# liuQuan98/EYOC

Measured on AMD Instinct MI355X. Metric: registered pairs/sec (30k-voxel KITTI pairs), higher is better.
Workload: dtype f32 (split16 products: fp32 storage/accumulation, 3 fp16 MFMAs on hi/lo-split operands per product); 1 GPU; 64 synthetic 30 cm KITTI-shaped pairs per step per GPU (mean 29894 voxels/cloud, ResUNetBN2C random-init, 5000-point NN, RANSAC 4000000 hypotheses/pair, planted inlier ratio 0.3, spconv math split16); parallelism=pairs sharded over 1 GPU(s), steps_in_flight=2

## Files before the change

### eyoc_amd/_lib.py

```python
from __future__ import annotations

import ctypes as C
import os
import threading

_HERE = os.path.dirname(os.path.abspath(__file__))
LIB_PATH = os.environ.get("EYOC_HIP_LIB") or os.path.join(_HERE, "lib", "libeyoc_hip.so")

MAX_LEVELS = 4
MAP_S1, MAP_DOWN, MAP_UP = 0, 1, 2


class MapsInfo(C.Structure):
    _fields_ = [("n_levels", C.c_int32), ("rows", C.c_int32 * MAX_LEVELS),
                ("pairs_s1", C.c_int64 * MAX_LEVELS), ("pairs_down", C.c_int64 * MAX_LEVELS),
                ("pairs_up", C.c_int64 * MAX_LEVELS), ("pairs_conv1", C.c_int64)]


class ModelDesc(C.Structure):
    _fields_ = [("in_channels", C.c_int32), ("out_channels", C.c_int32), ("conv1_kernel_size", C.c_int32),
                ("normalize_feature", C.c_int32), ("channels", C.c_int32 * 5), ("tr_channels", C.c_int32 * 5),
                ("bn_eps", C.c_float), ("expanded", C.c_int32)]


# ... 147 lines not shown
    "eyoc_split16_decode": (_i, [_vp, _vp, _i, _i, _i, _vp, _i, _vp]),
    "eyoc_model_set_math": (_i, [_vp, _i]),
    "eyoc_model_last_math": (_i, [_vp]),
    "eyoc_model_range_check": (_i, [_vp, _vp, C.POINTER(C.c_float)]),
    "eyoc_model_range_snapshot": (_i, [_vp, _vp, _vp]),
    "eyoc_model_set_progress_event": (_i, [_vp, _i, _vp]),
    "eyoc_model_set_probe": (_i, [_vp, _i]),
    "eyoc_spconv": (_i, [_vp, _vp, _i, _i, _vp, _i, _i, _vp, _i, _vp, _vp, _i, _i, _vp, _i, _vp]),
    "eyoc_spconv_sum": (_i, [_vp, _vp, _i, _i, _vp, _i, _i, _vp, _i, _vp, _i, _vp]),
    "eyoc_model_blob_floats": (_sz, [C.POINTER(ModelDesc)]),
    "eyoc_model_pack_host": (_i, [C.POINTER(ModelDesc), C.POINTER(LayerParams), _i, _vp, _sz]),
    "eyoc_model_create": (_i, [_vp, C.POINTER(ModelDesc), C.POINTER(LayerParams), _i, _vp, _sz, C.POINTER(_vp)]),
    "eyoc_model_blob_floats_in": (_sz, [C.POINTER(ModelDesc), _i]),
    "eyoc_model_pack_host_in": (_i, [C.POINTER(ModelDesc), C.POINTER(LayerParams), _i, _vp, _sz, _i]),
    "eyoc_model_create_in": (_i, [_vp, C.POINTER(ModelDesc), C.POINTER(LayerParams), _i, _vp, _sz, _i, C.POINTER(_vp)]),
    "eyoc_model_destroy": (_i, [_vp]),
    "eyoc_model_repack_workspace_bytes": (_sz, [_vp]),
    "eyoc_model_repack_device": (_i, [_vp, _vp, C.POINTER(LayerParams), _i, _vp, _sz, _vp]),
    "eyoc_model_fuse_tail": (_i, [_vp, _i]),
    "eyoc_model_workspace_bytes": (_sz, [_vp, _vp]),
    "eyoc_model_forward": (_i, [_vp, _vp, _vp, _vp, _vp, _vp, _sz, _vp]),
    "eyoc_model_workspace_bytes_rows": (_sz, [_vp, _vp, _i]),
    "eyoc_model_forward_rows": (_i, [_vp, _vp, _vp, _vp, _vp, _i, _vp, _vp, _sz, _vp]),
    "eyoc_model_sampled_tail": (_i, [_vp, _i]),
    "eyoc_model_num_layers": (_i, [_vp]),
    "eyoc_model_layer_work": (_i, [_vp, _vp, _vp, _vp, C.POINTER(C.c_char_p), C.POINTER(C.c_int64),
                                   C.POINTER(C.c_double), C.POINTER(C.c_double), C.POINTER(C.c_double)]),
    "eyoc_model_set_timing": (_i, [_vp, _i]),
    "eyoc_model_layer_ms": (_i, [_vp, C.POINTER(C.c_float)]),
    "eyoc_model_timing_slot": (_i, [_vp, _i]),
    "eyoc_bn_workspace_bytes": (_sz, [_i, _i]),
    "eyoc_bn_train_forward": (_i, [_vp, _vp, _i, _i, _i, _vp, _vp, C.c_float, _i, _vp, _i, _vp, _vp, _sz, _vp]),
    "eyoc_bn_train_forward_running": (_i, [_vp, _vp, _i, _i, _i, _vp, _vp, C.c_float, _i, _vp, _i, _vp, _vp, _vp, C.c_float, _vp, _sz, _vp]),
    "eyoc_bn_train_backward": (_i, [_vp, _vp, _i, _vp, _i, _vp, _i, _i, _i, _vp, _vp, C.c_float, _vp, _i, _vp, _vp, _vp, _sz, _vp]),
    "eyoc_in_chunk_rows": (_i, []),
    "eyoc_in_plan_bytes": (_sz, [_i, _i]),
    "eyoc_in_plan_layout": (_i, [_i, _i, C.POINTER(C.c_int64)]),
    "eyoc_in_plan_build": (_i, [_vp, _vp, _i, _i, _vp, _sz, _vp]),
    "eyoc_in_workspace_bytes": (_sz, [_i, _i, _i]),
    "eyoc_in_forward": (_i, [_vp, _vp, _i, _i, _i, _vp, _i, _vp, _vp, C.c_float, _i, _vp, _i, _vp, _i, _vp, _vp, _sz, _vp]),
    "eyoc_in_forward_split16": (_i, [_vp, _vp, _i, _i, _i, _vp, _i, _vp, _vp, C.c_float, _i, _vp, _i, _vp, _i, _vp, _vp, _vp, _sz, _vp]),
    "eyoc_in_backward": (_i, [_vp, _vp, _i, _vp, _i, _vp, _i, _i, _i, _vp, _i, _vp, _vp, C.c_float, _vp, _i, _vp, _i, _vp, _vp, _vp, _sz,
                              _vp]),
    "eyoc_maps_gather_window": (_i, [_vp, _vp, _i, _vp, _i, _vp, _vp]),
    "eyoc_maps_gather_window_internal": (_i, [_vp, _vp, _i, _vp, _i, _vp, _vp]),
    "eyoc_knn_prefilter": (_i, [_vp, _i]),
    "eyoc_spconv_select_up_kernel": (_i, [_vp, _i]),
    "eyoc_spconv_upc_min_rows": (_i, [_vp, _i]),
    "eyoc_spconv_upc_tile_rows": (_i, [_i, _i]),
    "eyoc_spconv_upc_bytes": (_sz, [_i]),
    "eyoc_spconv_upc_build": (_i, [_vp, _vp, _i, _vp, _vp, _vp]),
    "eyoc_spconv_upc": (_i, [_vp, _vp, _vp, _i, _i, _vp, _i, _i, _vp, _i, _vp, _i, _vp, _i, _i, _vp, _vp]),
    "eyoc_spconv_select_conv1_kernel": (_i, [_vp, _i]),
    "eyoc_knn1": (_i, [_vp, _vp, _vp, _i, C.POINTER(C.c_int32), C.POINTER(C.c_int32), _i, _i, _vp, _vp, _vp]),
    "eyoc_pdist": (_i, [_vp, _vp, _i, _vp, _i, _i, _i, _vp, _vp]),
    "eyoc_kabsch_batched": (_i, [_vp, _vp, _vp, _vp, _i, _i, _vp, _vp]),
    "eyoc_irls_quad": (_i, [_vp, _vp, _vp, _vp, _i, _i, _vp, _vp]),
    "eyoc_irls_quad_batched": (_i, [_vp, _vp, _vp, _vp, _vp, C.POINTER(C.c_int32), C.POINTER(C.c_int32), _i, _i, _vp, _vp]),
    "eyoc_valid_metrics_batched": (_i, [_vp, _vp, _vp, _vp, C.POINTER(C.c_int32), C.POINTER(C.c_int32), _vp, C.POINTER(C.c_int32), _i, _vp, _vp,
                                        C.c_double, C.c_double, _vp, _vp]),
    "eyoc_ransac": (_i, [_vp, _vp, _vp, _vp, _i, C.POINTER(RansacParams), _vp, _vp]),
    "eyoc_maps_select_orders": (_i, [_vp, _i, _i]),
    "eyoc_ransac_select_pruning": (_i, [_vp, _i]),
    "eyoc_ransac_select_generate": (_i, [_vp, _i]),
    "eyoc_knn_pack_targets": (_i, [_vp, _vp, C.POINTER(C.c_int32), _i, _i, _vp, _sz, _vp, _vp]),
    "eyoc_registration_accept_degenerate": (_i, [_vp, _i]),
    "eyoc_ransac_transform_store": (_i, [_vp, _i]),
    "eyoc_ransac_workspace_bytes": (_sz, [_vp, _i, _i, _i, _sz]),
    "eyoc_ransac_batched_ws": (_i, [_vp, _vp, _vp, _vp, C.POINTER(C.c_int32), C.POINTER(C.c_int32), _i,
                                    C.POINTER(RansacParams), _vp, _vp, _sz, _vp]),
    "eyoc_ransac_batched": (_i, [_vp, _vp, _vp, _vp, C.POINTER(C.c_int32), C.POINTER(C.c_int32), _i,
                                 C.POINTER(RansacParams), _vp, _vp]),
    "eyoc_sc2pcr_workspace_bytes": (_sz, [_i, C.POINTER(Sc2pcrParams)]),
    "eyoc_sc2pcr": (_i, [_vp, _vp, _vp, _i, C.POINTER(Sc2pcrParams), _vp, _vp, _vp, _sz, _vp]),
    "eyoc_sc2pcr_batched_workspace_bytes": (_sz, [_i, C.POINTER(Sc2pcrParams)]),
    "eyoc_sc2pcr_batched_workspace_bytes_n": (_sz, [_i, _i, C.POINTER(Sc2pcrParams)]),
    "eyoc_sc2pcr_set_shortlist_cap": (_i, [_vp, _i]),
    "eyoc_sc2pcr_set_dense_threshold": (_i, [_vp, _i]),
    "eyoc_sc2pcr_select_kernels": (_i, [_vp, _i]),
    "eyoc_sc2pcr_workspace_layout": (_i, [_i, C.POINTER(Sc2pcrParams), C.POINTER(Sc2pcrLayout)]),
    "eyoc_sc2pcr_batched": (_i, [_vp, _vp, _vp, C.POINTER(C.c_int32), _i, C.POINTER(Sc2pcrParams), _vp, _vp, _i, _vp, _sz,
                                 _vp]),
    "eyoc_icp_workspace_bytes": (_sz, [_i, _i, _i]),
    "eyoc_icp_batched": (_i, [_vp, _vp, _vp, C.POINTER(C.c_int32), C.POINTER(C.c_int32), _i, _vp, C.POINTER(IcpParams), _vp, _vp,
                              _vp, _sz, _vp]),
    "eyoc_icp_correspondences": (_i, [_vp, _vp, _vp, C.POINTER(C.c_int32), C.POINTER(C.c_int32), _i, _vp, C.c_double, _vp, _vp,
                                      _vp, _vp, _sz, _vp]),
    "eyoc_posed_nn_grid_workspace_bytes": (_sz, [_i, _i, _i]),
    "eyoc_posed_nn_grid": (_i, [_vp, _vp, _vp, C.POINTER(C.c_int32), C.POINTER(C.c_int32), _i, _vp, C.c_float, _vp, C.POINTER(C.c_int32), _vp,
                                _vp, _vp, _vp, _sz, _vp]),
    "eyoc_radius_matches_workspace_bytes": (_sz, [_i, _i, _i]),
    "eyoc_radius_matches_count": (_i, [_vp, _vp, _vp, C.POINTER(C.c_int32), C.POINTER(C.c_int32), _i, _vp, C.c_double, _i, _vp, _vp,
                                       _vp, _sz, _vp]),
    "eyoc_radius_matches_fill": (_i, [_vp, _vp, _vp, C.POINTER(C.c_int32), C.POINTER(C.c_int32), _i, _vp, C.c_double, _i, _vp, _vp,
                                      C.c_int64, _vp, _vp, _vp, _sz, _vp]),
    "eyoc_cloud_centroids_workspace_bytes": (_sz, [_i, _i]),
    "eyoc_cloud_centroids": (_i, [_vp, _vp, _i, C.POINTER(C.c_int64), _i, _i, _vp, _vp, _sz, _vp]),
    "eyoc_augment_poses": (_i, [_vp, _vp, _vp, _vp, _vp, _i, _vp, _vp, _vp]),
    "eyoc_voxelize_batched_posed_workspace_bytes": (_sz, [_i, _i]),
    "eyoc_voxelize_batched_posed": (_i, [_vp, _vp, _i, C.POINTER(C.c_int64), _i, _i, _vp, _vp, C.c_double, _i, _vp, _vp, _vp,
                                         C.POINTER(C.c_int64), _vp, _sz, _vp, _vp]),
    "eyoc_hcloss_workspace_bytes": (_sz, [_i, _i, _i, _i, _i]),
    "eyoc_hcloss_workspace_layout": (_i, [_i, _i, _i, _i, _i, C.POINTER(HclossLayout)]),
    "eyoc_hcloss_forward": (_i, [_vp, _vp, _i, _vp, _i, _i, _vp, _i, _vp, _i, _vp, _i, _vp, _i, C.c_float, C.c_float, _vp, _vp, _sz, _vp]),
    "eyoc_hcloss_backward": (_i, [_vp, _vp, _i, _vp, _i, _i, _vp, _i, _vp, _i, _vp, _i, _vp, _i, C.c_float, C.c_float, _vp, _vp, _vp, _vp,
                                  _vp, _sz, _vp]),
# ... 153 lines not shown
```

### eyoc_amd/csrc/common.h

```cpp
#pragma once
#include <hip/hip_runtime.h>

#include <cstdarg>
#include <cstdint>
#include <cstdio>
#include <cstring>
#include <string>
#include <vector>

#include "../../include/eyoc_hip.h"

namespace eyoc {

void set_error(const char* fmt, ...);

#define EYOC_CHECK_HIP(expr)                                                               \
  do {                                                                                     \
    hipError_t _e = (expr);                                                                \
    if (_e != hipSuccess) {                                                                \
      eyoc::set_error("%s failed: %s (%s:%d)", #expr, hipGetErrorString(_e), __FILE__,    \
                      __LINE__);                                                           \
      return EYOC_ERR_HIP;                                                                 \
    }                                                                                      \
  } while (0)

#define EYOC_REQUIRE(cond, code, ...)  \
  do {                                 \
    if (!(cond)) {                     \
      eyoc::set_error(__VA_ARGS__);    \
      return (code);                   \
    }                                  \
  } while (0)

inline size_t align_up(size_t v, size_t a = 256) { return (v + a - 1) / a * a; }
inline int cdiv(long long a, long long b) { return (int)((a + b - 1) / b); }

struct Carver {
  char* base;
  size_t off = 0, cap;
  Carver(void* p, size_t bytes) : base((char*)p), cap(bytes) {}
  template <typename T>
  T* take(size_t count) {
    size_t o = align_up(off);
    off = o + count * sizeof(T);
    return (T*)(base ? base + o : nullptr);
  }
  bool ok() const { return off <= cap; }
};

}

struct eyoc_ctx {
  int device = 0;
  void* scratch = nullptr;
  size_t scratch_bytes = 0;
  void* pinned = nullptr;
  size_t pinned_bytes = 0;
  int ensure_scratch(size_t bytes, hipStream_t st);
  hipStream_t scratch_owner = nullptr;
  bool scratch_owned = false;
  hipEvent_t scratch_ev = nullptr;
  static constexpr int POOL = 8;
  hipStream_t pool[POOL] = {};
  hipEvent_t pool_done[POOL] = {};
  hipEvent_t pool_fork = nullptr;
  bool pool_ready = false;
  int ensure_pool();
  bool ransac_attr_set = false, sc2_attr_set = false;
  bool up_attr_set[2] = {false, false};
  int zorder_kbits = 17, zorder_bbits = 10;
  int sc2_list_cap = 1024, sc2_dense_x = 0;
  int sc2_legacy = 0;
  uint32_t fault_dup[32] = {}, fault_range[32] = {};
  struct Knobs {
    int maps_order_min_rows = 65536;
    int maps_window_shift = 18;
    int maps_s1_order = 1, maps_down_order = 0;
    int maps_internal_order = -1;
    int maps_lazy_tables = 1, maps_fused_levels = 1;
    int knn_prefilter = 1;
    int fuse_tail = 2;
    int sampled_tail = 1;
    int spconv_kernel = -1;
    int split16_kernel = 1;
    int up_kernel = 2;
    int s1_wide = 1;
    int st128_wide = 1;
    int down_kernel = 1;
    int upc_min_rows = 1 << 17;
    int conv1_kernel = 1;
    int st_group = 1;
    int st_variant = 1;
    int st_split_below = 1024;
    int st_cg_local = 1;
    int st_ksplit = 1;
    int ransac_store = 1 << 20;
    int ransac_prune = 2;
    int ransac_generate = 1;
    int accept_degenerate = 0;
  } knobs;
};
inline const eyoc_ctx::Knobs& knobs_of(const eyoc_ctx* ctx) {
  static const eyoc_ctx::Knobs defaults;
  return ctx ? ctx->knobs : defaults;
}

namespace eyoc {

constexpr unsigned long long KEY_EMPTY = 0xFFFFFFFFFFFFFFFFull;
constexpr int COORD_BIAS = 1 << 17;
constexpr int VAL_UNSET = 0x7F7F7F7F;

struct HashTable {
  unsigned long long* keys;
  int* vals;
  unsigned int mask;
};

__host__ __device__ inline unsigned long long pack_key(int b, int x, int y, int z) {
  return ((unsigned long long)(unsigned)b << 54) |
         ((unsigned long long)((unsigned)(x + COORD_BIAS) & 0x3FFFFu) << 36) |
         ((unsigned long long)((unsigned)(y + COORD_BIAS) & 0x3FFFFu) << 18) |
         ((unsigned long long)((unsigned)(z + COORD_BIAS) & 0x3FFFFu));
}

__host__ __device__ inline unsigned int hash_key(unsigned long long k) {
  k ^= k >> 33;
  k *= 0xff51afd7ed558ccdull;
  k ^= k >> 33;
  k *= 0xc4ceb9fe1a85ec53ull;
  k ^= k >> 33;
  return (unsigned int)k;
}

__device__ inline int hash_lookup(const HashTable& t, unsigned long long key) {
  unsigned int s = hash_key(key) & t.mask;
  for (unsigned int probes = 0; probes <= t.mask; ++probes) {
    unsigned long long k = t.keys[s];
    if (k == key) return t.vals[s];
    if (k == KEY_EMPTY) return -1;
    s = (s + 1) & t.mask;
  }
  return -1;
// ... 53 lines not shown
```

### eyoc_amd/csrc/spconv.hip

```cpp
#include <cmath>
#include <cstdlib>
#include <type_traits>

#include "spconv.h"

using namespace eyoc;

namespace {

typedef float f32x4 __attribute__((ext_vector_type(4)));

constexpr int KMAX = 27;

#ifdef EYOC_TRACE
constexpr int TRACE_STAMPS = 512, TRACE_WAVES = 8, TRACE_BLOCKS = 8;
__device__ unsigned long long g_trace[TRACE_BLOCKS * TRACE_WAVES * TRACE_STAMPS];
#define TR_DECL const int tr_blk = (blockIdx.x >= 300 && blockIdx.x < 300 + TRACE_BLOCKS && blockIdx.y == 0) ? (int)blockIdx.x - 300 : -1; int tr_n = 0
#define TR() do { if (tr_blk >= 0 && (threadIdx.x & 63) == 0 && tr_n < TRACE_STAMPS) \
    g_trace[(tr_blk * TRACE_WAVES + (threadIdx.x >> 6)) * TRACE_STAMPS + tr_n++] = __builtin_readcyclecounter(); } while (0)
#else
#define TR_DECL
#define TR()
#endif

// ... 890 lines not shown
    }
#if CONV1_BF_ABL == 4
    for (int c0 = 0; c0 < min(nq, 16); c0 += 16) {
#else
    for (int c0 = 0; c0 < nq; c0 += 16) {
#endif
      const int idx = c0 + j;
      const bool ok = idx < nq;
      const int pl = lpar[q][ok ? idx : 0];
      const int o = f0 + (int)lrow[q][ok ? idx : 0];
      const int sl = inv[pl];
      const int ew = (sl >> 6) * 16 + (sl & 15), ec = (sl >> 4) & 3;
      f32x4 acc[NT];
#pragma unroll
      for (int t = 0; t < NT; ++t) acc[t] = f32x4{0.f, 0.f, 0.f, 0.f};
#pragma unroll
      for (int t = 0; t < NS7; ++t) {
        const int kc = 4 * t + g;
        int slot = ZSLOT;
        if (kc < 27) {
          const int e0 = ent[(kc * 64 + ew) * 4 + ec] >> 6;
          if (e0 != ST_UMAX) slot = e0;
          else if (n_pass > 1) {
            const int e1 = loc[((size_t)(27 + kc) * 64 + ew) * 4 + ec] >> 6;
            if (e1 != ST_UMAX) slot = ST_UMAX + e1;
          }
        }
        const half8_t vh = *reinterpret_cast<const half8_t*>(&cfh[slot][0]);
        const half8_t vl = *reinterpret_cast<const half8_t*>(&cfl[slot][0]);
#pragma unroll
        for (int tt = 0; tt < NT; ++tt) {
          acc[tt] = __builtin_amdgcn_mfma_f32_16x16x32_f16(wh[t][tt], vh, acc[tt], 0, 0, 0);
          acc[tt] = __builtin_amdgcn_mfma_f32_16x16x32_f16(wh[t][tt], vl, acc[tt], 0, 0, 0);
          acc[tt] = __builtin_amdgcn_mfma_f32_16x16x32_f16(wl[t][tt], vh, acc[tt], 0, 0, 0);
        }
      }
      if (ok) {
        float* dst = a.out + (size_t)o * a.ld_out;
#pragma unroll
        for (int t = 0; t < NT; ++t) {
          const int ch0 = 16 * t + 4 * g;
          const float4 v = make_float4(acc[t][0] * iwsc + bias4[t].x, acc[t][1] * iwsc + bias4[t].y,
                                       acc[t][2] * iwsc + bias4[t].z, acc[t][3] * iwsc + bias4[t].w);
          split16_track(mx, v);
          if (a.out_split) split16_store4(dst, ch0, v);
          else *reinterpret_cast<float4*>(dst + ch0) = v;
        }
      }
    }
  }
  if (a.out_split) split16_report(a.range, mx);
}

int launch_conv1(const Conv1Args& a, hipStream_t st) {
  EYOC_REQUIRE(a.ks == 1 || a.ks == 3 || a.ks == 5 || a.ks == 7, EYOC_ERR_INVALID, "conv1: kernel size %d", a.ks);
  EYOC_REQUIRE(a.cin >= 1 && a.cin * a.cout <= 8192, EYOC_ERR_INVALID, "conv1: C_in %d x C_out %d too large", a.cin, a.cout);
  EYOC_REQUIRE(a.ld_out % 4 == 0, EYOC_ERR_INVALID, "conv1: ld_out must be a multiple of 4");
  if (a.n == 0) return EYOC_OK;
  dim3 grid(cdiv(a.n, 256));
  const size_t tree_lds = (size_t)a.ks * a.ks * a.ks * a.cin * (a.cout + 4) * sizeof(float);
  if (conv1_walks_octree(a)) {
    if (knobs_of(a.ctx).conv1_kernel != 2 && a.cin == 1 && a.cout == 32 && a.out_split && a.ks * a.ks * a.ks < 128 && !a.in_perm) {
      if (a.local1 && knobs_of(a.ctx).conv1_kernel == 1) {
        hipLaunchKernelGGL(conv1_bf_kernel, dim3(cdiv(a.nc, ST_TILE)), dim3(256), 0, st, a);
        EYOC_CHECK_HIP(hipGetLastError());
        return EYOC_OK;
      }
      const int wgs = cdiv(a.n, 64);
      hipLaunchKernelGGL(conv1_mfma_kernel, dim3(wgs < 2560 ? wgs : 2560), dim3(256), 0, st, a);
      EYOC_CHECK_HIP(hipGetLastError());
      return EYOC_OK;
    }
    switch (a.cout) {
      case 32: hipLaunchKernelGGL(conv1_tree_kernel<32>, grid, dim3(256), tree_lds, st, a); break;
      case 64: hipLaunchKernelGGL(conv1_tree_kernel<64>, grid, dim3(256), tree_lds, st, a); break;
      case 128: hipLaunchKernelGGL(conv1_tree_kernel<128>, grid, dim3(256), tree_lds, st, a); break;
      default:
        set_error("conv1: C_out %d not in {32,64,128}", a.cout);
        return EYOC_ERR_INVALID;
    }
    EYOC_CHECK_HIP(hipGetLastError());
    return EYOC_OK;
  }
  switch (a.cout) {
    case 32: hipLaunchKernelGGL(conv1_kernel<32>, grid, dim3(256), 0, st, a); break;
    case 64: hipLaunchKernelGGL(conv1_kernel<64>, grid, dim3(256), 0, st, a); break;
    case 128: hipLaunchKernelGGL(conv1_kernel<128>, grid, dim3(256), 0, st, a); break;
    default:
      set_error("conv1: C_out %d not in {32,64,128}", a.cout);
      return EYOC_ERR_INVALID;
  }
  EYOC_CHECK_HIP(hipGetLastError());
  return EYOC_OK;
}

}

#ifdef EYOC_TRACE
extern "C" int eyoc_debug_trace(unsigned long long* out_host, size_t count) {
  return (int)hipMemcpyFromSymbol(out_host, HIP_SYMBOL(g_trace), count * sizeof(unsigned long long));
}
#endif

extern "C" {

size_t eyoc_spconv_packed_floats(int K, int cin, int cout) { return (size_t)K * cin * cout; }

int eyoc_spconv_select_kernel(eyoc_ctx* ctx, int mode) {
  if (!ctx) return -2;
  const int prev = ctx->knobs.spconv_kernel;
  ctx->knobs.spconv_kernel = mode;
  return prev;
}

int eyoc_spconv_pack_weights(const float* w, const float* scale, int K, int cin, int cout, float* packed) {
// ... 110 lines not shown
}
int eyoc_spconv_st_ksplit(eyoc_ctx* ctx, int on) {
  if (!ctx) return -1;
  const int prev = ctx->knobs.st_ksplit;
  if (on == 0 || on == 1) ctx->knobs.st_ksplit = on;
  if (on == 2 || on == 3) ctx->knobs.st_cg_local = on - 2;
  return prev;
}

int eyoc_spconv_select_up_kernel(eyoc_ctx* ctx, int on) {
  if (!ctx) return -1;
  const int prev = ctx->knobs.up_kernel;
  if (on >= 0 && on <= 2) ctx->knobs.up_kernel = on;
  return prev;
}

int eyoc_spconv_upc_min_rows(eyoc_ctx* ctx, int rows) {
  if (!ctx) return -1;
  const int prev = ctx->knobs.upc_min_rows;
  if (rows >= 0) ctx->knobs.upc_min_rows = rows;
  return prev;
}

int eyoc_spconv_upc_tile_rows(int odd_axes, int rows) { return eyoc::upc_set_tile_rows(odd_axes, rows); }

size_t eyoc_spconv_upc_bytes(int n_out) { return n_out < 0 ? 0 : eyoc::upc_kept_bytes(n_out) + eyoc::upc_scratch_bytes(n_out) + 512; }

int eyoc_spconv_upc_build(eyoc_ctx* ctx, const int32_t* nbr_dev, int n_out, void* ws_dev, int32_t* info_host, void* stream) {
  EYOC_REQUIRE(ctx && nbr_dev && ws_dev && n_out >= 0 && ((uintptr_t)ws_dev & 255) == 0, EYOC_ERR_INVALID, "eyoc_spconv_upc_build: bad argument");
  unsigned char* ws = (unsigned char*)ws_dev;
  if (int rc = eyoc::build_upc(nbr_dev, nullptr, 1, n_out, ws, ws + ((eyoc::upc_kept_bytes(n_out) + 255) & ~(size_t)255), (hipStream_t)stream)) return rc;
  if (info_host) {
    EYOC_CHECK_HIP(hipMemcpyAsync(info_host, ws, 19 * sizeof(int32_t), hipMemcpyDeviceToHost, (hipStream_t)stream));
    EYOC_CHECK_HIP(hipStreamSynchronize((hipStream_t)stream));
  }
  return EYOC_OK;
}

int eyoc_spconv_upc(eyoc_ctx* ctx, const int32_t* nbr_dev, const void* ws_dev, int n_out, int n_in, const float* in_dev, int ld_in, int cin,
                    const float* wpacked_dev, int cout, const float* bias_dev, int relu, float* out_dev, int ld_out, int out_split,
                    const float* out_scale_dev, void* stream) {
  EYOC_REQUIRE(ctx && nbr_dev && ws_dev, EYOC_ERR_INVALID, "eyoc_spconv_upc: NULL argument");
  SpconvArgs a;
  a.nbr = nbr_dev; a.K = 27; a.n_out = n_out; a.n_in = n_in; a.in = in_dev; a.ld_in = ld_in; a.cin = cin; a.w = wpacked_dev;
  a.cout = cout; a.bias = bias_dev; a.res = nullptr; a.ld_res = 0; a.relu = relu; a.l2norm = 0;
  a.out = out_dev; a.ld_out = ld_out; a.math = 1; a.out_split = out_split; a.out_scale = out_scale_dev;
  a.local_upc = (const unsigned char*)ws_dev; a.ctx = ctx;
  return launch_spconv(a, (hipStream_t)stream);
}

int eyoc_spconv_select_conv1_kernel(eyoc_ctx* ctx, int on) {
  if (!ctx) return -1;
  const int prev = ctx->knobs.conv1_kernel;
  if (on >= 0 && on <= 2) ctx->knobs.conv1_kernel = on;
  return prev;
}

int eyoc_spconv_select_st_kernel(eyoc_ctx* ctx, int variant) {
  if (!ctx) return -1;
  const int prev = ctx->knobs.st_variant;
  if (variant >= 0 && variant < eyoc::st_variants()) ctx->knobs.st_variant = variant;
  return prev;
}

int eyoc_spconv_st_split_below(eyoc_ctx* ctx, int workgroups) {
  if (!ctx) return -1;
  const int prev = ctx->knobs.st_split_below;
  if (workgroups >= 0) ctx->knobs.st_split_below = workgroups;
  return prev;
}

int eyoc_spconv_select_split16_kernel(eyoc_ctx* ctx, int mode) {
  if (!ctx) return -1;
  const int prev = ctx->knobs.split16_kernel;
  if (mode >= 0 && mode <= 2) ctx->knobs.split16_kernel = mode;
  return prev;
}

int eyoc_spconv_ex(eyoc_ctx* ctx, const int32_t* nbr_dev, int K, int n_out, int n_in, const float* in_dev, int ld_in, int cin,
                   const float* wpacked_dev, int cout, const float* bias_dev, const float* res_dev, int ld_res, int relu,
                   float* out_dev, int ld_out, int math, int out_split, const float* out_scale_dev, void* stream) {
  EYOC_REQUIRE(ctx, EYOC_ERR_INVALID, "eyoc_spconv_ex: NULL ctx");
  EYOC_REQUIRE(math == 0 || math == 1, EYOC_ERR_INVALID, "eyoc_spconv_ex: math %d", math);
  SpconvArgs a;
  a.nbr = nbr_dev; a.K = K; a.n_out = n_out; a.n_in = n_in; a.in = in_dev; a.ld_in = ld_in; a.cin = cin; a.w = wpacked_dev;
  a.cout = cout; a.bias = bias_dev; a.res = res_dev; a.ld_res = ld_res; a.relu = relu; a.l2norm = 0;
  a.out = out_dev; a.ld_out = ld_out; a.math = math; a.out_split = out_split; a.out_scale = out_scale_dev; a.ctx = ctx;
  return launch_spconv(a, (hipStream_t)stream);
}

int eyoc_split16_encode(eyoc_ctx* ctx, const float* in_dev, int n, int c, int ld_in, float* out_dev, int ld_out, void* stream) {
  EYOC_REQUIRE(ctx && in_dev && out_dev && n >= 0 && c > 0 && c % 32 == 0 && ld_in % 4 == 0 && ld_out % 32 == 0, EYOC_ERR_INVALID,
               "eyoc_split16_encode: bad argument (c %d must be a multiple of 32)", c);
  if (n) hipLaunchKernelGGL(k_split16_encode, dim3(cdiv((long long)n * (c / 4), 256)), dim3(256), 0, (hipStream_t)stream, in_dev, n, c, ld_in, out_dev, ld_out);
  EYOC_CHECK_HIP(hipGetLastError());
  return EYOC_OK;
}

int eyoc_split16_decode(eyoc_ctx* ctx, const float* in_dev, int n, int c, int ld_in, float* out_dev, int ld_out, void* stream) {
  EYOC_REQUIRE(ctx && in_dev && out_dev && n >= 0 && c > 0 && c % 32 == 0 && ld_in % 32 == 0 && ld_out % 4 == 0, EYOC_ERR_INVALID,
               "eyoc_split16_decode: bad argument (c %d must be a multiple of 32)", c);
  if (n) hipLaunchKernelGGL(k_split16_decode, dim3(cdiv((long long)n * (c / 4), 256)), dim3(256), 0, (hipStream_t)stream, in_dev, n, c, ld_in, out_dev, ld_out);
  EYOC_CHECK_HIP(hipGetLastError());
  return EYOC_OK;
}

int eyoc_spconv(eyoc_ctx* ctx, const int32_t* nbr_dev, int K, int n_out, const float* in_dev, int ld_in, int cin,
// ... 22 lines not shown
```

### include/eyoc_hip.h

```cpp
#ifndef EYOC_HIP_H
#define EYOC_HIP_H

#include <stddef.h>
#include <stdint.h>

#ifdef __cplusplus
extern "C" {
#endif

typedef struct eyoc_ctx eyoc_ctx;
typedef struct eyoc_maps eyoc_maps;
typedef struct eyoc_model eyoc_model;

typedef enum {
  EYOC_OK = 0,
  EYOC_ERR_INVALID = -1,
  EYOC_ERR_HIP = -2,
  EYOC_ERR_WORKSPACE = -3,
  EYOC_ERR_DUPLICATE = -4,
  EYOC_ERR_RANGE = -5
} eyoc_status;

#define EYOC_MAX_LEVELS 4
#define EYOC_VERSION 111
// ... 28 lines not shown
int eyoc_maps_internal_order(eyoc_ctx* ctx, int mode);
int eyoc_maps_lazy_tables(eyoc_ctx* ctx, int on);
int eyoc_maps_fused_levels(eyoc_ctx* ctx, int on);
int eyoc_spconv_select_down_kernel(eyoc_ctx* ctx, int mode);
const int32_t* eyoc_maps_row_order(const eyoc_maps* maps);
int eyoc_maps_copy_row_order(const eyoc_maps* maps, int32_t* out_dev, void* stream);
int eyoc_maps_rows(const eyoc_maps* maps, int level);
const int32_t* eyoc_maps_coords(const eyoc_maps* maps, int level);
const int32_t* eyoc_maps_table(const eyoc_maps* maps, int kind, int level);
int eyoc_maps_copy_coords(const eyoc_maps* maps, int level, int32_t* out_dev, void* stream);
int eyoc_maps_copy_table(const eyoc_maps* maps, int kind, int level, int32_t* out_dev, void* stream);
int eyoc_maps_info(eyoc_ctx* ctx, const eyoc_maps* maps, int conv1_kernel_size, void* stream,
                   eyoc_maps_info_t* info);

size_t eyoc_voxelize_workspace_bytes(int n_points);
int eyoc_voxelize(eyoc_ctx* ctx, const float* xyz_dev, int n_points, int stride, float voxel_size, int batch_index,
                  int32_t* sel_dev, int32_t* coords_dev, int* n_out, void* workspace_dev, size_t workspace_bytes,
                  void* stream);

size_t eyoc_voxelize_batched_workspace_bytes(int n_points_total, int n_clouds);
int eyoc_voxelize_batched(eyoc_ctx* ctx, const float* xyz_dev, int stride, const int64_t* point_offsets, int n_clouds,
                          int n_points, float voxel_size, int batch_base, int32_t* sel_dev, int32_t* coords_dev,
                          float* xyz_out_dev, int64_t* voxel_offsets, void* workspace_dev, size_t workspace_bytes,
                          void* stream);
size_t eyoc_voxelize_batched_isolating_workspace_bytes(int n_points_total, int n_clouds);
int eyoc_voxelize_batched_isolating(eyoc_ctx* ctx, const float* xyz_dev, int stride, const int64_t* point_offsets, int n_clouds,
                                    int n_points, float voxel_size, int batch_base, int32_t* sel_dev, int32_t* coords_dev,
                                    float* xyz_out_dev, int64_t* voxel_offsets, void* workspace_dev, size_t workspace_bytes,
                                    void* stream, int32_t* cloud_faults);

size_t eyoc_batch_drop_workspace_bytes(int n_rows);
int eyoc_batch_drop(eyoc_ctx* ctx, const int32_t* coords_dev, const float* feats_dev, int n_rows, int c, const uint32_t* drop_mask,
                    int32_t* coords_out_dev, float* feats_out_dev, int32_t* row_map_dev, int* n_kept, int32_t* kept_per_batch,
                    void* workspace_dev, size_t workspace_bytes, void* stream);
int eyoc_remap_rows(eyoc_ctx* ctx, const int64_t* idx_dev, int m, const int32_t* row_map_dev, int n_rows, int64_t* out_dev,
                    void* stream);

size_t eyoc_spconv_packed_floats(int K, int cin, int cout);
int eyoc_spconv_pack_weights(const float* w_host , const float* scale_host ,
                             int K, int cin, int cout, float* packed_host);
int eyoc_spconv(eyoc_ctx* ctx, const int32_t* nbr_dev, int K, int n_out, const float* in_dev,
                int ld_in, int cin, const float* wpacked_dev, int cout, const float* bias_dev,
                const float* res_dev, int ld_res, int relu, float* out_dev, int ld_out, void* stream);
int eyoc_spconv_select_split16_kernel(eyoc_ctx* ctx, int mode);
int eyoc_spconv_select_up_kernel(eyoc_ctx* ctx, int on);
int eyoc_spconv_upc_min_rows(eyoc_ctx* ctx, int rows);
int eyoc_spconv_upc_tile_rows(int odd_axes, int rows);
size_t eyoc_spconv_upc_bytes(int n_out);
int eyoc_spconv_upc_build(eyoc_ctx* ctx, const int32_t* nbr_dev, int n_out, void* ws_dev, int32_t* info_host, void* stream);
int eyoc_spconv_upc(eyoc_ctx* ctx, const int32_t* nbr_dev, const void* ws_dev, int n_out, int n_in, const float* in_dev, int ld_in,
                    int cin, const float* wpacked_dev, int cout, const float* bias_dev, int relu, float* out_dev, int ld_out,
                    int out_split, const float* out_scale_dev, void* stream);
int eyoc_spconv_select_conv1_kernel(eyoc_ctx* ctx, int on);
int eyoc_spconv_select_st_kernel(eyoc_ctx* ctx, int variant);
int eyoc_spconv_st_split_below(eyoc_ctx* ctx, int workgroups);
int eyoc_spconv_st_group_rows(eyoc_ctx* ctx, int on);
int eyoc_spconv_st_ksplit(eyoc_ctx* ctx, int on);
size_t eyoc_spconv_local_rulebook_bytes(int n_out);
int eyoc_spconv_build_local_rulebook(eyoc_ctx* ctx, const int32_t* nbr_dev, int K, int n_out, void* out_dev,
                                     int32_t* overflow_dev, void* stream);
int eyoc_spconv_staged(eyoc_ctx* ctx, const int32_t* nbr_dev, const void* local_dev, int n_out, int n_in, const float* in_dev,
                       int ld_in, int cin, const float* wpacked_dev, int cout, const float* bias_dev, const float* res_dev,
                       int ld_res, int relu, float* out_dev, int ld_out, int out_split, const float* out_scale_dev, void* stream);
int eyoc_spconv_build_local_rulebook128(eyoc_ctx* ctx, const int32_t* nbr_dev, int K, int n_out, void* out_dev,
                                        int32_t* overflow_dev, void* stream);
int eyoc_spconv_staged128(eyoc_ctx* ctx, const int32_t* nbr_dev, const void* local_dev, int n_out, int n_in, const float* in_dev,
                          int ld_in, int cin, const float* wpacked_dev, int cout, const float* bias_dev, const float* res_dev,
                          int ld_res, int relu, float* out_dev, int ld_out, int out_split, const float* out_scale_dev, void* stream);
int eyoc_spconv_pack_weights_split16(const float* w_host, const float* scale_host, int K, int cin, int cout,
                                     float* packed_host, float* out_scale_host);
int eyoc_spconv_ex(eyoc_ctx* ctx, const int32_t* nbr_dev, int K, int n_out, int n_in, const float* in_dev, int ld_in, int cin,
                   const float* wpacked_dev, int cout, const float* bias_dev, const float* res_dev, int ld_res, int relu,
                   float* out_dev, int ld_out, int math, int out_split, const float* out_scale_dev, void* stream);
int eyoc_split16_encode(eyoc_ctx* ctx, const float* in_dev, int n, int c, int ld_in, float* out_dev, int ld_out, void* stream);
int eyoc_split16_decode(eyoc_ctx* ctx, const float* in_dev, int n, int c, int ld_in, float* out_dev, int ld_out, void* stream);
int eyoc_spconv_sum(eyoc_ctx* ctx, const int32_t* nbr_dev, int K, int n_out, const float* in_dev, int ld_in, int cin,
                    const float* wpacked_dev, int cout, float* out_dev, int ld_out, void* stream);
int eyoc_spconv_pack_weights_transposed(const float* w_host , int K, int cin, int cout, int mirror,
                                        float* packed_host);
size_t eyoc_spconv_grad_weight_workspace_bytes(int K, int n_out, int cin, int cout);
int eyoc_spconv_grad_weight(eyoc_ctx* ctx, const int32_t* nbr_dev, int K, int n_out, const float* in_dev, int ld_in, int cin,
                            const float* dout_dev, int ld_dout, int cout, float* dw_dev, void* workspace_dev,
                            size_t workspace_bytes, void* stream);
int eyoc_spconv_select_kernel(eyoc_ctx* ctx, int mode);

typedef struct {
  int32_t in_channels, out_channels, conv1_kernel_size, normalize_feature;
  int32_t channels[5];
  int32_t tr_channels[5];
  float bn_eps;
  int32_t expanded;
} eyoc_model_desc;

typedef struct {
  const char* name;
  const float* kernel;
  int32_t K, cin, cout;
  const float* bias;
  const float* bn_weight;
  const float* bn_bias;
  const float* bn_mean;
  const float* bn_var;
} eyoc_layer_params;

size_t eyoc_model_blob_floats(const eyoc_model_desc* desc);
int eyoc_model_pack_host(const eyoc_model_desc* desc, const eyoc_layer_params* layers, int n_layers,
// ... 338 lines not shown
```

Measured before the change: 3479 pairs/s.

## Add persistent double-buffered conv1 kernel with one workgroup per CU

Adds a persistent conv1 kernel for the 1-to-32-channel first convolution. Each workgroup is sized to one per CU, loops over tiles and double-buffers tile metadata and split-fp16 input features in LDS, so gathers for the next tile overlap the MFMA work on the current one. Weights are split and loaded into registers once per workgroup, not once per tile. This becomes the default conv1 path and adds a knob for the workgroup count. The cost is lower occupancy, one workgroup per CU with a large LDS footprint, and more complex barriers.

```diff
diff --git a/eyoc_amd/_lib.py b/eyoc_amd/_lib.py
--- a/eyoc_amd/_lib.py
+++ b/eyoc_amd/_lib.py
@@ -223,6 +223,7 @@
     "eyoc_spconv_upc_build": (_i, [_vp, _vp, _i, _vp, _vp, _vp]),
     "eyoc_spconv_upc": (_i, [_vp, _vp, _vp, _i, _i, _vp, _i, _i, _vp, _i, _vp, _i, _vp, _i, _i, _vp, _vp]),
     "eyoc_spconv_select_conv1_kernel": (_i, [_vp, _i]),
+    "eyoc_spconv_conv1_workgroups": (_i, [_vp, _i]),
     "eyoc_knn1": (_i, [_vp, _vp, _vp, _i, C.POINTER(C.c_int32), C.POINTER(C.c_int32), _i, _i, _vp, _vp, _vp]),
     "eyoc_pdist": (_i, [_vp, _vp, _i, _vp, _i, _i, _i, _vp, _vp]),
     "eyoc_kabsch_batched": (_i, [_vp, _vp, _vp, _vp, _i, _i, _vp, _vp]),
diff --git a/eyoc_amd/csrc/common.h b/eyoc_amd/csrc/common.h
--- a/eyoc_amd/csrc/common.h
+++ b/eyoc_amd/csrc/common.h
@@ -68,6 +68,8 @@
   int ensure_pool();
   bool ransac_attr_set = false, sc2_attr_set = false;
   bool up_attr_set[2] = {false, false};
+  bool conv1p_attr_set = false;
+  int n_cus = 0;
   int zorder_kbits = 17, zorder_bbits = 10;
   int sc2_list_cap = 1024, sc2_dense_x = 0;
   int sc2_legacy = 0;
@@ -88,7 +90,8 @@
     int st128_wide = 1;
     int down_kernel = 1;
     int upc_min_rows = 1 << 17;
-    int conv1_kernel = 1;
+    int conv1_kernel = 3;
+    int conv1_workgroups = 0;
     int st_group = 1;
     int st_variant = 1;
     int st_split_below = 1024;
diff --git a/eyoc_amd/csrc/spconv.hip b/eyoc_amd/csrc/spconv.hip
--- a/eyoc_amd/csrc/spconv.hip
+++ b/eyoc_amd/csrc/spconv.hip
@@ -966,6 +966,240 @@
   if (a.out_split) split16_report(a.range, mx);
 }
 
+struct alignas(16) Conv1Tile {
+  static constexpr int NSLOT = ST_NPASS * ST_UMAX + 1;
+  _Float16 cfh[NSLOT][8], cfl[NSLOT][8];
+  unsigned short ent[27 * 64 * 4];
+  unsigned short lrow[8][ST_TILE];
+  unsigned char lpar[8][ST_TILE];
+  unsigned char inv[ST_TILE];
+  int ctot[8];
+  int f0, pad[3];
+};
+struct alignas(16) Conv1Shared {
+  Conv1Tile tile[2];
+  _Float16 w5h[128][32], w5l[128][32];
+  signed char ktab[8][216];
+  float bias[32];
+  int ccnt[8][4], f0h[2], pad[2];
+};
+static_assert(sizeof(Conv1Shared) <= 160 * 1024, "conv1_bfp_kernel: one workgroup per CU, within its LDS");
+extern __shared__ __attribute__((aligned(16))) unsigned char conv1p_smem[];
+
+__global__ __launch_bounds__(512, 1) void conv1_bfp_kernel(Conv1Args a, int n_tiles) {
+  constexpr int COUT = 32, NT = COUT / 16, NS7 = 7;
+  constexpr int NSLOT = Conv1Tile::NSLOT, ZSLOT = NSLOT - 1;
+  constexpr int NS = (NSLOT + 511) / 512;
+  constexpr int NENT = 27 * 64 * 4 * 2 / 16;
+  Conv1Shared& S = *reinterpret_cast<Conv1Shared*>(conv1p_smem);
+  const int tid = threadIdx.x, lane = tid & 63, wave = tid >> 6;
+  const int j = lane & 15, g = lane >> 4;
+  const int K = a.ks * a.ks * a.ks, r = a.ks / 2;
+  const int G = gridDim.x;
+  const int4* __restrict__ child4 = reinterpret_cast<const int4*>(a.children);
+  const float* __restrict__ fin = a.in;
+  int tn = blockIdx.x;
+  int nu_n, un[NS];
+  {
+    const unsigned char* lr = a.local1 + (size_t)tn * ST_LR_BYTES;
+    nu_n = *reinterpret_cast<const int*>(lr);
+#pragma unroll
+    for (int i = 0; i < NS; ++i) un[i] = reinterpret_cast<const int*>(lr + 16)[min(tid + 512 * i, ST_UCAP - 1)];
+  }
+  for (int e = tid; e < 8 * 216; e += 512) {
+    const int cls = e / 216, kc = (e % 216) / 8, cs = e % 8;
+    const int dx = 2 * (kc % 3 - 1) + (cs & 1) - (cls & 1), dy = 2 * ((kc / 3) % 3 - 1) + ((cs >> 1) & 1) - ((cls >> 1) & 1),
+              dz = 2 * (kc / 9 - 1) + (cs >> 2) - (cls >> 2);
+    const bool in = dx >= -r && dx <= r && dy >= -r && dy <= r && dz >= -r && dz <= r;
+    S.ktab[cls][kc * 8 + cs] = (signed char)(in ? (dx + r) + a.ks * (dy + r) + a.ks * a.ks * (dz + r) : 127);
+  }
+  {
+    const float wsc = a.wscale ? a.wscale[0] : 256.0f;
+    for (int e = tid; e < 128 * COUT; e += 512) {
+      const int k = e / COUT;
+      const float w = k < K ? a.w[e] * wsc : 0.0f;
+      const _Float16 h = (_Float16)w;
+      (&S.w5h[0][0])[e] = h;
+      (&S.w5l[0][0])[e] = (_Float16)(w - (float)h);
+    }
+  }
+  if (tid < 32) {
+    const int b = tid >> 4, e = tid & 15;
+    (e < 8 ? S.tile[b].cfh[ZSLOT][e] : S.tile[b].cfl[ZSLOT][e - 8]) = (_Float16)0.f;
+  }
+  if (tid >= 64 && tid < 64 + COUT) S.bias[tid - 64] = a.bias[tid - 64];
+  __syncthreads();
+  half8_t wh[NS7][NT], wl[NS7][NT];
+#pragma unroll
+  for (int t = 0; t < NS7; ++t) {
+    const int kc = 4 * t + g;
+#pragma unroll
+    for (int i = 0; i < 8; ++i) {
+      const int kp = kc < 27 ? (int)S.ktab[wave][kc * 8 + i] : 127;
+#pragma unroll
+      for (int tt = 0; tt < NT; ++tt) {
+        wh[t][tt][i] = S.w5h[kp][16 * tt + j];
+        wl[t][tt][i] = S.w5l[kp][16 * tt + j];
+      }
+    }
+  }
+  const float iwsc = a.wscale ? a.wscale[1] : 1.0f / 256.0f;
+  float mx = 0.f;
+  typedef float f32x4 __attribute__((ext_vector_type(4)));
+  int tc = -1, nu_c = 0;
+  for (int it = 0;; ++it) {
+    const Conv1Tile& B = S.tile[it & 1];
+    Conv1Tile& N = S.tile[(it & 1) ^ 1];
+    const unsigned char* lrn = a.local1 + (size_t)min(tn, n_tiles - 1) * ST_LR_BYTES;
+    int4 c0[NS], c1[NS];
+#pragma unroll
+    for (int i = 0; i < NS; ++i) {
+      const int u = tid + 512 * i < nu_n ? min(max(un[i], 0), a.nc - 1) : 0;
+      c0[i] = child4[2 * (size_t)u];
+      c1[i] = child4[2 * (size_t)u + 1];
+    }
+    const uint4* esrc = reinterpret_cast<const uint4*>(lrn + ST_LOC_OFF);
+    const uint4 en0 = esrc[tid], en1 = esrc[min(tid + 512, NENT - 1)];
+    const unsigned int invw = reinterpret_cast<const unsigned int*>(lrn + ST_INV_OFF)[lane];
+    const int nq = tc >= 0 ? B.ctot[wave] : 0;
+    const int f0 = B.f0;
+    const int n_pass = nu_c > ST_UMAX ? 2 : 1;
+    const unsigned short* __restrict__ loc = reinterpret_cast<const unsigned short*>(a.local1 + (size_t)max(tc, 0) * ST_LR_BYTES + ST_LOC_OFF);
+    auto chunk = [&](const int c0r) __attribute__((always_inline)) {
+      const int idx = c0r + j;
+      const bool ok = idx < nq;
+      const int pl = B.lpar[wave][ok ? idx : 0];
+      const int o = f0 + (int)B.lrow[wave][ok ? idx : 0];
+      const int sl = B.inv[pl];
+      const int ew = (sl >> 6) * 16 + (sl & 15), ec = (sl >> 4) & 3;
+      f32x4 acc[NT];
+#pragma unroll
+      for (int t = 0; t < NT; ++t) acc[t] = f32x4{0.f, 0.f, 0.f, 0.f};
+      int slot[NS7];
+#pragma unroll
+      for (int t = 0; t < NS7; ++t) {
+        const int kc = min(4 * t + g, 26);
+        const int e0 = B.ent[(kc * 64 + ew) * 4 + ec] >> 6;
+        slot[t] = 4 * t + g < 27 ? e0 : -1;
+      }
+      if (n_pass > 1) {
+#pragma unroll
+        for (int t = 0; t < NS7; ++t) {
+          const int e1 = loc[((27 + min(4 * t + g, 26)) * 64 + ew) * 4 + ec] >> 6;
+          slot[t] = slot[t] != ST_UMAX ? slot[t] : e1 != ST_UMAX ? ST_UMAX + e1 : -1;
+        }
+      } else {
+#pragma unroll
+        for (int t = 0; t < NS7; ++t) slot[t] = slot[t] == ST_UMAX ? -1 : slot[t];
+      }
+#pragma unroll
+      for (int t = 0; t < NS7; ++t) {
+        const int sl_t = slot[t] < 0 ? ZSLOT : slot[t];
+        const half8_t vh = *reinterpret_cast<const half8_t*>(&B.cfh[sl_t][0]);
+        const half8_t vl = *reinterpret_cast<const half8_t*>(&B.cfl[sl_t][0]);
+#pragma unroll
+        for (int tt = 0; tt < NT; ++tt) {
+          acc[tt] = __builtin_amdgcn_mfma_f32_16x16x32_f16(wh[t][tt], vh, acc[tt], 0, 0, 0);
+          acc[tt] = __builtin_amdgcn_mfma_f32_16x16x32_f16(wh[t][tt], vl, acc[tt], 0, 0, 0);
+          acc[tt] = __builtin_amdgcn_mfma_f32_16x16x32_f16(wl[t][tt], vh, acc[tt], 0, 0, 0);
+        }
+      }
+      if (ok) {
+        float* dst = a.out + (size_t)o * a.ld_out;
+#pragma unroll
+        for (int t = 0; t < NT; ++t) {
+          const int ch0 = 16 * t + 4 * g;
+          const float4 b4 = *reinterpret_cast<const float4*>(&S.bias[ch0]);
+          const float4 v = make_float4(acc[t][0] * iwsc + b4.x, acc[t][1] * iwsc + b4.y, acc[t][2] * iwsc + b4.z, acc[t][3] * iwsc + b4.w);
+          split16_track(mx, v);
+          if (a.out_split) split16_store4(dst, ch0, v);
+          else *reinterpret_cast<float4*>(dst + ch0) = v;
+        }
+      }
+    };
+    const int nch = (nq + 15) >> 4, nch0 = (nch + 1) >> 1;
+    for (int c = 0; c < nch0; ++c) chunk(16 * c);
+    reinterpret_cast<uint4*>(N.ent)[tid] = en0;
+    if (tid + 512 < NENT) reinterpret_cast<uint4*>(N.ent)[tid + 512] = en1;
+    if (tid < 64) reinterpret_cast<unsigned int*>(N.inv)[tid] = invw;
+    float f[NS][8];
+    unsigned int vmask = 0;
+#pragma unroll
+    for (int i = 0; i < NS; ++i) {
+      const int v[8] = {c0[i].x, c0[i].y, c0[i].z, c0[i].w, c1[i].x, c1[i].y, c1[i].z, c1[i].w};
+#pragma unroll
+      for (int q = 0; q < 8; ++q) {
+        f[i][q] = fin[max(v[q], 0)];
+        vmask |= v[q] >= 0 ? 1u << (8 * i + q) : 0u;
+      }
+    }
+    const int pl_own = tid & 255, hf = tid >> 8;
+    const int prow = min(tn, n_tiles - 1) * ST_TILE + pl_own;
+    const int4 own = child4[2 * (size_t)min(prow, a.nc - 1) + hf];
+    int nu_2, un2[NS];
+    {
+      const unsigned char* lr2 = a.local1 + (size_t)min(tn + G, n_tiles - 1) * ST_LR_BYTES;
+      nu_2 = *reinterpret_cast<const int*>(lr2);
+#pragma unroll
+      for (int i = 0; i < NS; ++i) un2[i] = reinterpret_cast<const int*>(lr2 + 16)[min(tid + 512 * i, ST_UCAP - 1)];
+    }
+    for (int c = nch0; c < nch; ++c) chunk(16 * c);
+#pragma unroll
+    for (int i = 0; i < NS; ++i) {
+      const int s = tid + 512 * i;
+      if (s < nu_n) {
+        half8_t h8, l8;
+#pragma unroll
+        for (int q = 0; q < 8; ++q) {
+          const float x = (vmask >> (8 * i + q)) & 1u ? f[i][q] : 0.f;
+          h8[q] = (_Float16)x;
+          l8[q] = (_Float16)(x - (float)h8[q]);
+        }
+        *reinterpret_cast<half8_t*>(&N.cfh[s][0]) = h8;
+        *reinterpret_cast<half8_t*>(&N.cfl[s][0]) = l8;
+      }
+    }
+    int v[4] = {own.x, own.y, own.z, own.w};
+    if (prow >= a.nc) v[0] = v[1] = v[2] = v[3] = -1;
+    if (pl_own == 0) {
+      int m = a.n;
+#pragma unroll
+      for (int q = 0; q < 4; ++q) if (v[q] >= 0 && v[q] < m) m = v[q];
+      S.f0h[hf] = m;
+    }
+    unsigned long long bm[4];
+#pragma unroll
+    for (int q = 0; q < 4; ++q) {
+      bm[q] = __ballot(v[q] >= 0);
+      if (lane == 0) S.ccnt[4 * hf + q][wave & 3] = __popcll(bm[q]);
+    }
+    lds_barrier();
+    const int f0n = min(S.f0h[0], S.f0h[1]);
+#pragma unroll
+    for (int q = 0; q < 4; ++q) {
+      const int cls = 4 * hf + q;
+      int base = 0;
+      for (int w = 0; w < (wave & 3); ++w) base += S.ccnt[cls][w];
+      if (v[q] >= 0) {
+        const int pos = base + (int)__builtin_amdgcn_mbcnt_hi((unsigned int)(bm[q] >> 32), __builtin_amdgcn_mbcnt_lo((unsigned int)bm[q], 0u));
+        N.lrow[cls][pos] = (unsigned short)(v[q] - f0n);
+        N.lpar[cls][pos] = (unsigned char)pl_own;
+      }
+    }
+    if (tid < 8) N.ctot[tid] = S.ccnt[tid][0] + S.ccnt[tid][1] + S.ccnt[tid][2] + S.ccnt[tid][3];
+    if (tid == 0) N.f0 = f0n;
+    lds_barrier();
+    tc = tn;
+    nu_c = nu_n;
+    if (tc >= n_tiles) break;
+    tn += G;
+    nu_n = nu_2;
+#pragma unroll
+    for (int i = 0; i < NS; ++i) un[i] = un2[i];
+  }
+  if (a.out_split) split16_report(a.range, mx);
+}
+
 int launch_conv1(const Conv1Args& a, hipStream_t st) {
   EYOC_REQUIRE(a.ks == 1 || a.ks == 3 || a.ks == 5 || a.ks == 7, EYOC_ERR_INVALID, "conv1: kernel size %d", a.ks);
   EYOC_REQUIRE(a.cin >= 1 && a.cin * a.cout <= 8192, EYOC_ERR_INVALID, "conv1: C_in %d x C_out %d too large", a.cin, a.cout);
@@ -975,6 +1209,25 @@
   const size_t tree_lds = (size_t)a.ks * a.ks * a.ks * a.cin * (a.cout + 4) * sizeof(float);
   if (conv1_walks_octree(a)) {
     if (knobs_of(a.ctx).conv1_kernel != 2 && a.cin == 1 && a.cout == 32 && a.out_split && a.ks * a.ks * a.ks < 128 && !a.in_perm) {
+      if (a.local1 && knobs_of(a.ctx).conv1_kernel == 3) {
+        eyoc_ctx* ctx = const_cast<eyoc_ctx*>(a.ctx);
+        int cus = ctx ? ctx->n_cus : 0;
+        if (cus <= 0) {
+          int dev = 0;
+          EYOC_CHECK_HIP(hipGetDevice(&dev));
+          EYOC_CHECK_HIP(hipDeviceGetAttribute(&cus, hipDeviceAttributeMultiprocessorCount, dev));
+          EYOC_REQUIRE(cus > 0, EYOC_ERR_INVALID, "conv1: device reports %d compute units", cus);
+          if (ctx) ctx->n_cus = cus;
+        }
+        if (!ctx || !ctx->conv1p_attr_set) {
+          EYOC_CHECK_HIP(hipFuncSetAttribute(reinterpret_cast<const void*>(conv1_bfp_kernel), hipFuncAttributeMaxDynamicSharedMemorySize, (int)sizeof(Conv1Shared)));
+          if (ctx) ctx->conv1p_attr_set = true;
+        }
+        const int n_tiles = cdiv(a.nc, ST_TILE), want = knobs_of(a.ctx).conv1_workgroups > 0 ? knobs_of(a.ctx).conv1_workgroups : cus;
+        hipLaunchKernelGGL(conv1_bfp_kernel, dim3(n_tiles < want ? n_tiles : want), dim3(512), sizeof(Conv1Shared), st, a, n_tiles);
+        EYOC_CHECK_HIP(hipGetLastError());
+        return EYOC_OK;
+      }
       if (a.local1 && knobs_of(a.ctx).conv1_kernel == 1) {
         hipLaunchKernelGGL(conv1_bf_kernel, dim3(cdiv(a.nc, ST_TILE)), dim3(256), 0, st, a);
         EYOC_CHECK_HIP(hipGetLastError());
@@ -1191,7 +1444,14 @@
 int eyoc_spconv_select_conv1_kernel(eyoc_ctx* ctx, int on) {
   if (!ctx) return -1;
   const int prev = ctx->knobs.conv1_kernel;
-  if (on >= 0 && on <= 2) ctx->knobs.conv1_kernel = on;
+  if (on >= 0 && on <= 3) ctx->knobs.conv1_kernel = on;
+  return prev;
+}
+
+int eyoc_spconv_conv1_workgroups(eyoc_ctx* ctx, int workgroups) {
+  if (!ctx) return -1;
+  const int prev = ctx->knobs.conv1_workgroups;
+  if (workgroups >= 0) ctx->knobs.conv1_workgroups = workgroups;
   return prev;
 }
 
diff --git a/include/eyoc_hip.h b/include/eyoc_hip.h
--- a/include/eyoc_hip.h
+++ b/include/eyoc_hip.h
@@ -104,6 +104,7 @@
                     int cin, const float* wpacked_dev, int cout, const float* bias_dev, int relu, float* out_dev, int ld_out,
                     int out_split, const float* out_scale_dev, void* stream);
 int eyoc_spconv_select_conv1_kernel(eyoc_ctx* ctx, int on);
+int eyoc_spconv_conv1_workgroups(eyoc_ctx* ctx, int workgroups);
 int eyoc_spconv_select_st_kernel(eyoc_ctx* ctx, int variant);
 int eyoc_spconv_st_split_below(eyoc_ctx* ctx, int workgroups);
 int eyoc_spconv_st_group_rows(eyoc_ctx* ctx, int on);
```

Measured after the change: 3543 pairs/s (median of 6 runs). 1.02x the previous value.
